# pkuyzy/TLC-GNN

Measured on NVIDIA B200. Metric: vicinity_pd_pi_per_sec, higher is better.
Workload: dtype f64

## Files before the change

### tlc-gnn_b200/csrc/k1t_sssp_table.cu

```cuda
#include <cstdlib>

#include <cstdio>
#include <cstring>

#include "tlc_common.cuh"

namespace tlc {
namespace {

__global__ void sssp_mark_kernel(const int32_t* __restrict__ targets, int64_t E, int node_mode, GraphView g, SsspTables tb) {
  const int64_t total = 2 * E;
  for (int64_t i = blockIdx.x * (int64_t)blockDim.x + threadIdx.x; i < total; i += (int64_t)gridDim.x * blockDim.x) {
    if (node_mode && (i & 1)) continue;
    const int32_t x = targets[i];
    if (x < 0 || x >= g.N || g.rowptr[x + 1] == g.rowptr[x]) continue;
    if (tb.state[x] == 0 && atomicCAS(&tb.state[x], 0, 1) == 0) tb.list[atomicAdd(tb.count, 1)] = x;
  }
}

__global__ void sssp_mark_all_kernel(GraphView g, SsspTables tb) {
  for (int x = blockIdx.x * blockDim.x + threadIdx.x; x < g.N; x += gridDim.x * blockDim.x) {
    if (g.rowptr[x + 1] == g.rowptr[x]) continue;
    if (tb.state[x] == 0 && atomicCAS(&tb.state[x], 0, 1) == 0) tb.list[atomicAdd(tb.count, 1)] = x;
  }
}

constexpr int BQ = 2048;
struct BuildShared {
  int32_t q[BQ];
  int32_t qn, qhead;
  unsigned long long dmin;
  int32_t any;
};

__global__ void __launch_bounds__(1024) sssp_build_kernel(GraphView g, SsspTables tb, const uint32_t* __restrict__ ball_cache,
                                                          const float* __restrict__ gminw, double* __restrict__ pw_scratch,
                                                          int plain) {
  extern __shared__ __align__(16) unsigned long long bsm[];
  __shared__ BuildShared sh;
  const int N = g.N, W = (N + 31) / 32;
  const int tid = threadIdx.x, nt = blockDim.x, lane = tid & 31, wid = tid >> 5, nw = nt >> 5;
  unsigned long long* dist = bsm;
  int32_t* par = reinterpret_cast<int32_t*>(bsm + N);
  uint32_t* ball = reinterpret_cast<uint32_t*>(par + N);
  uint8_t* state = reinterpret_cast<uint8_t*>(ball + W);
  double* pw = pw_scratch + (size_t)blockIdx.x * N;
  const int cnt = *tb.count;
  for (int idx = blockIdx.x; idx < cnt; idx += gridDim.x) {
    const int32_t root = tb.list[idx];
    __syncthreads();
    for (int x = tid; x < N; x += nt) { dist[x] = INF_BITS; state[x] = 0; par[x] = -1; }
    for (int w = tid; w < W; w += nt) ball[w] = ball_cache[(size_t)root * W + w];
    __syncthreads();
    if (tid == 0) { dist[root] = 0ull; state[root] = 1; }
    __syncthreads();
    for (int phase = 0; phase < 2 * N + 2; phase++) {
      if (tid == 0) { sh.dmin = INF_BITS; sh.qn = 0; sh.qhead = 0; }
      __syncthreads();
      unsigned long long lm = INF_BITS;
      for (int x = tid; x < N; x += nt) if (state[x] == 1) { const unsigned long long d = dist[x]; lm = d < lm ? d : lm; }
      lm = warp_min_u64(lm);
      if (lane == 0 && lm != INF_BITS) atomicMin(&sh.dmin, lm);
      __syncthreads();
      const unsigned long long dminb = sh.dmin;
      if (dminb == INF_BITS) break;
      const double dmin = __longlong_as_double((long long)dminb);
      for (int x = tid; x < N; x += nt) {
        if (state[x] != 1) continue;
        if (__longlong_as_double((long long)dist[x]) <= __dadd_rn(dmin, (double)gminw[x])) {
          const int pos = atomicAdd(&sh.qn, 1);
          if (pos < BQ) { state[x] = 2; sh.q[pos] = x; }
        }
      }
      __syncthreads();
      const int qn = min(sh.qn, BQ);
      for (;;) {
        int i = 0;
        if (lane == 0) i = atomicAdd(&sh.qhead, 1);
        i = __shfl_sync(0xffffffffu, i, 0);
        if (i >= qn) break;
        const int x = sh.q[i];
        const double dx = __longlong_as_double((long long)dist[x]);
        const int a = g.rowptr[x], b = g.rowptr[x + 1];
        for (int e = a + lane; e < b; e += 32) {
          const int y = g.col[e];
          if (!test_bit(ball, y)) continue;
          const unsigned long long tbv = (unsigned long long)__double_as_longlong(__dadd_rn(dx, __dadd_rn(g.kappa[e], 1.0)));
          if (tbv < dist[y]) { atomicMin(&dist[y], tbv); if (state[y] == 0) state[y] = 1; }
        }
      }
      __syncthreads();
    }
    __syncthreads();
    for (int x = wid; x < N; x += nw) {
      const unsigned long long dxb = dist[x];
      if (x == root || dxb == INF_BITS) continue;
      const int a = g.rowptr[x], b = g.rowptr[x + 1];
      for (int e0 = a; e0 < b; e0 += 32) {
        const int e = e0 + lane;
        bool hit = false;
        double w = 0.0;
        int y = 0;
        if (e < b) {
          y = g.col[e];
          w = __dadd_rn(g.kappa[e], 1.0);
          const unsigned long long dyb = dist[y];
          hit = dyb != INF_BITS && (unsigned long long)__double_as_longlong(__dadd_rn(__longlong_as_double((long long)dyb), w)) == dxb;
        }
        const unsigned bal = __ballot_sync(0xffffffffu, hit);
        if (bal) {
          if (lane == __ffs(bal) - 1) { par[x] = y; pw[x] = w; }
          break;
        }
      }
    }
    __threadfence_block();
    __syncthreads();
    double* Drow = tb.D + (size_t)root * N;
    double* Qrow = tb.Q + (size_t)root * N;
    int32_t* Prow = tb.P + (size_t)root * N;
    double* Wrow = tb.PW + (size_t)root * N;
    for (int x = tid; x < N; x += nt) {
      const unsigned long long dxb = dist[x];
      Drow[x] = __longlong_as_double((long long)dxb);
      Prow[x] = par[x];
      Wrow[x] = par[x] >= 0 ? pw[x] : 0.0;
      double res;
      if (x == root) res = 0.0;
      else if (dxb == INF_BITS || par[x] < 0) res = NO_PATH_DIST;
      else {
        PySum ps{0.0, 0.0, 0};
        int y = x, guard = 0;
        while (y != root && guard++ <= N) { pysum_add(ps, pw[y], plain != 0); y = par[y]; }
        res = pysum_get(ps, plain != 0);
      }
      Qrow[x] = res;
    }
    __syncthreads();
    if (tid == 0) { __threadfence(); tb.state[root] = 2; }
  }
}

struct TableShared {
  double redd[32];
  int32_t wsum[33];
  int32_t ninv;
  int32_t nextra;
  int32_t dinv;
  int32_t nia;
  int32_t any;
};
#ifdef T1_PROFILE
__device__ unsigned long long g_t1prof[24];
#define TPROF(i) do { if (tid == 0) { const long long tnow_ = clock64(); atomicAdd(&g_t1prof[i], (unsigned long long)(tnow_ - tprev_)); tprev_ = tnow_; } } while (0)
#else
#define TPROF(i) do { } while (0)
#endif


__global__ void __launch_bounds__(1024) filtration_table_kernel(Params p, ChunkView c, int t0, int cap, GraphView g,
                                                                const uint32_t* __restrict__ ball_cache, SsspTables tb, int W) {
  extern __shared__ __align__(16) unsigned long long dynt[];
  __shared__ TableShared sh;
  const int t = t0 + blockIdx.x;
  const int tid = threadIdx.x, nt = blockDim.x, lane = tid & 31, wid = tid >> 5, nw = nt >> 5;
  const bool node_mode = p.mode == TLC_MODE_NODE;
  const int64_t vo = c.voff[t];
  const int N = g.N;
  unsigned long long* dist = dynt;
  uint16_t* parl = reinterpret_cast<uint16_t*>(dynt + cap);
  uint8_t* cls = reinterpret_cast<uint8_t*>(parl + cap);
  uint32_t* bm = reinterpret_cast<uint32_t*>(reinterpret_cast<unsigned char*>(dynt) + (size_t)cap * 11);
  uint16_t* lid = reinterpret_cast<uint16_t*>(bm + 2 * W);

#ifdef T1_PROFILE
  long long tprev_ = clock64();
#endif
  const int64_t ti = c.tidx[t];
  const int32_t u = c.tgt[2 * ti], v = c.tgt[2 * ti + 1];
  if (unknown_target(g, u, v, node_mode)) {
    if (tid == 0) { c.tn[t] = 0; c.tnp[t] = 0; c.tnpos[t] = 0; c.tnneg[t] = 0; c.tlu[t] = -1; c.tlv[t] = -1;
                    c.tstatus[t] = TLC_ST_UNKNOWN_NODE; }
    return;
  }
  const int n = graph_row_bitmap(c, t, ball_cache, W, u, v, node_mode, bm, sh.wsum);
  {
    uint32_t* l32 = reinterpret_cast<uint32_t*>(lid);
    for (int i = tid; i < (N + 1) / 2; i += nt) l32[i] = 0xffffffffu;
  }
  __syncthreads();
  for (int w = wid; w < W; w += nw) {
    const uint32_t bits = bm[w];
    if (!((bits >> lane) & 1u)) continue;
    const int lx = (int)bm[W + w] + __popc(bits & lanemask_lt());
    const int32_t x = w * 32 + lane;
    const int32_t ra = g.rowptr[x];
    c.vert[vo + lx] = x;
    c.astart[vo + lx] = ra;
    c.adeg[vo + lx] = g.rowptr[x + 1] - ra;
    lid[x] = (uint16_t)lx;
  }
  const int lu = bitmap_rank(bm, W, u);
  const int lv = node_mode ? lu : bitmap_rank(bm, W, v);
  uint8_t st0 = (lu >= 0 && lv >= 0) ? TLC_ST_OK : TLC_ST_TRIVIAL;
  if (n == 0 || (node_mode && n == 1)) st0 = TLC_ST_EMPTY;
  if (tid == 0) {
    c.tn[t] = n; c.tlu[t] = lu; c.tlv[t] = lv; c.tstatus[t] = st0;
    if (c.count_m) c.tm[t] = 0;
    c.tnp[t] = 0; c.tnpos[t] = 0; c.tnneg[t] = 0; c.tncls[t] = 0;
  }
  __syncthreads();
      TPROF(0);
  if (n == 0 || st0 > TLC_ST_TRIVIAL) return;

  const int32_t* __restrict__ vert = c.vert + vo;
  double* d1 = c.d1 + vo;
  double* d2 = c.d2 + vo;
  double* fval = c.fval + vo;
  int32_t* hint = c.neg + vo;
  int32_t* hint0 = c.vcls + vo;
  int32_t* inv = c.vs0 + vo;
  int32_t* extra = c.vs1 + vo;
  int32_t* bpos = c.vs2 + vo;
  uint32_t* iap = reinterpret_cast<uint32_t*>(c.vord + vo);
  int32_t* iaq = c.vrank + vo;
  uint2* ia2 = reinterpret_cast<uint2*>(c.v64a + vo);
  uint2* ia3 = reinterpret_cast<uint2*>(c.v64c + vo);
  uint2* ia4 = reinterpret_cast<uint2*>(c.fval + vo);
  const bool roots_in = lu >= 0 && lv >= 0;
  const bool plain = (p.flags & TLC_F_SUM_PLAIN) != 0;
  const bool two = roots_in && !node_mode && lu != lv;
  constexpr uint8_t UNKNOWN = 0, VALID = 1, INVALID = 2, UNREACH = 3;

  if (!roots_in) {
    for (int x = tid; x < n; x += nt) { d1[x] = NO_PATH_DIST; d2[x] = NO_PATH_DIST; hint[x] = -1; hint0[x] = -1; }
  } else {
    for (int r = 0; r < (two ? 2 : 1); r++) {
      const int root = r == 0 ? lu : lv;
      const int32_t groot = r == 0 ? u : v;
      const double* __restrict__ Drow = tb.D + (size_t)groot * N;
      const double* __restrict__ Qrow = tb.Q + (size_t)groot * N;
      const double* __restrict__ Wrow = tb.PW + (size_t)groot * N;
      const int32_t* __restrict__ Prow = tb.P + (size_t)groot * N;
      double* out = r == 0 ? d1 : d2;
      int32_t* hnt = r == 0 ? hint0 : hint;
      if (tid == 0) { sh.ninv = 0; sh.nextra = 0; sh.dinv = 0; sh.nia = 0; }
      for (int x = tid; x < n; x += nt) {
        const int32_t gx = vert[x];
        uint8_t cl;
        uint16_t pl = 0xffff;
        if (x == root) cl = VALID;
        else {
          const int32_t gp = Prow[gx];
          pl = gp >= 0 ? lid[gp] : (uint16_t)0xffff;
          cl = pl == 0xffff ? INVALID : UNKNOWN;
        }
        cls[x] = cl; parl[x] = pl;
        dist[x] = (unsigned long long)__double_as_longlong(Drow[gx]);
        if (r == 0) { hint[x] = -1; hint0[x] = -1; }
      }
      __syncthreads();
      TPROF(1);
      for (int round = 0; round <= n; round++) {
        int ch = 0;
        for (int x = tid; x < n; x += nt) {
          if (cls[x] != UNKNOWN) continue;
          const uint8_t pc = cls[parl[x]];
          if (pc != UNKNOWN) { cls[x] = pc; ch = 1; }
          else ch = 1;
        }
        if (!__syncthreads_or(ch)) break;
      }
      TPROF(2);
      for (int x0 = 0; x0 < n; x0 += nt) {
        const int x = x0 + tid;
        const bool iv = x < n && cls[x] == INVALID;
        const unsigned bal = __ballot_sync(0xffffffffu, iv);
        int base = 0;
        if (bal && lane == 0) base = atomicAdd(&sh.ninv, __popc(bal));
        base = __shfl_sync(0xffffffffu, base, 0);
        if (iv) {
          const int32_t gx = vert[x];
          inv[base + __popc(bal & lanemask_lt())] = x;
          dist[x] = INF_BITS; bpos[x] = 0x7fffffff;
          atomicAdd(&sh.dinv, g.rowptr[gx + 1] - g.rowptr[gx]);
        }
      }
      __syncthreads();
      TPROF(3);
      const int ninv = sh.ninv;
      int chunk = min(512, max(32, ((sh.dinv / (nt / 2) + 31) / 32) * 32));
      while (sh.dinv / chunk > n / 2) chunk *= 2;
      for (int i = tid; i < ninv; i += nt) {
        const int32_t gx = vert[inv[i]];
        const int cnt = (g.rowptr[gx + 1] - g.rowptr[gx] + chunk - 1) / chunk;
        if (cnt > 1) {
          const int at = atomicAdd(&sh.nextra, cnt - 1);
          for (int j = 1; j < cnt; j++) extra[at + j - 1] = (inv[i] << 12) | j;
        }
      }
      __syncthreads();
      TPROF(4);
      const int nextra = sh.nextra, nitems = ninv + nextra;
      const int l8 = lane & 7, grp = tid >> 3, ngrp = nt >> 3;
      const unsigned gm = 0xffu << (lane & 24);
      constexpr int ITEM_RESCAN = 1 << 30;
      auto item_bounds = [&](int i, int& x, int& a, int& b, bool flagged_only) {
        const int raw = i < ninv ? inv[i] : extra[i - ninv];
        const int pk = i < ninv ? ((raw & 0xffff) << 12) : (raw & (ITEM_RESCAN - 1));
        x = pk >> 12;
        const int ra = c.astart[vo + x];
        a = ra + (pk & 4095) * chunk;
        b = min(ra + c.adeg[vo + x], a + chunk);
        if (flagged_only && !(raw & ITEM_RESCAN)) b = a;
      };
      auto ia_put = [&](int k, uint32_t pr, int pos) {
        if (k < n) { iap[k] = pr; iaq[k] = pos; }
        else if (k < 2 * n) ia2[k - n] = make_uint2(pr, (uint32_t)pos);
        else if (k < 3 * n) ia3[k - 2 * n] = make_uint2(pr, (uint32_t)pos);
        else if (k < 4 * n) ia4[k - 3 * n] = make_uint2(pr, (uint32_t)pos);
      };
      auto ia_get = [&](int k, uint32_t& pr, int& pos) {
        if (k < n) { pr = iap[k]; pos = iaq[k]; return; }
        const uint2 v2 = k < 2 * n ? ia2[k - n] : k < 3 * n ? ia3[k - 2 * n] : ia4[k - 3 * n];
        pr = v2.x; pos = (int)v2.y;
      };
      const int capw = (4 * n) / nw;
      int cntw = 0;
      auto relax_rows = [&](bool first) -> int {
        int ch = 0;
        for (int kb = 0; kb * ngrp < nitems; kb += 8) {
          int mx = 0, ma = 0, mb = 0;
          { const int itl = (kb + l8) * ngrp + grp; if (itl < nitems) item_bounds(itl, mx, ma, mb, !first); }
          for (int j = 0; j < 8; j++) {
            const int x = __shfl_sync(gm, mx, j, 8), a = __shfl_sync(gm, ma, j, 8), b = __shfl_sync(gm, mb, j, 8);
            int trips = (b - a + 31) >> 5;
            trips = max(trips, __shfl_xor_sync(0xffffffffu, trips, 8));
            trips = max(trips, __shfl_xor_sync(0xffffffffu, trips, 16));
            unsigned long long best = INF_BITS;
            for (int t5 = 0; t5 < trips; t5++) {
              const int e0 = a + l8 + 32 * t5;
              uint4 rc[4];
// ... 55 lines not shown
          ewt[i] = __hiloint2double((int)rc.w, (int)rc.z);
        }
      }
#ifdef T1_PROFILE
      long long tlr0_ = clock64();
      int nrounds_ = 0;
#endif
      for (int round = 1; round <= ninv + 1; round++) {
        int ch = 0;
#ifdef T1_PROFILE
        nrounds_++;
#endif
#pragma unroll
        for (int i = 0; i < 4; i++) {
          if (epr[i] == 0xffffffffu) continue;
          const int x = (int)(epr[i] >> 16), ly = (int)(epr[i] & 0xffffu);
          const unsigned long long dyb = dist[ly], dxb = dist[x];
          if (dyb != INF_BITS) {
            const unsigned long long cand = (unsigned long long)__double_as_longlong(__dadd_rn(__longlong_as_double((long long)dyb), ewt[i]));
            if (cand < dxb && cand < atomicMin(&dist[x], cand)) ch = 1;
          }
          if (dxb != INF_BITS) {
            const unsigned long long c2 = (unsigned long long)__double_as_longlong(__dadd_rn(__longlong_as_double((long long)dxb), ewt[i]));
            if (c2 < dyb && c2 < atomicMin(&dist[ly], c2)) ch = 1;
          }
        }
        for (int k = lane + 128; k < nlist; k += 32) {
          uint32_t pr; int pos;
          ia_get(wid * capw + k, pr, pos);
          const int x = (int)(pr >> 16), ly = (int)(pr & 0xffffu);
          const unsigned long long dyb = dist[ly], dxb = dist[x];
          if (dyb == INF_BITS && dxb == INF_BITS) continue;
          const uint4 rc = __ldg(g.rec + pos);
          const double w = __hiloint2double((int)rc.w, (int)rc.z);
          if (dyb != INF_BITS) {
            const unsigned long long cand = (unsigned long long)__double_as_longlong(__dadd_rn(__longlong_as_double((long long)dyb), w));
            if (cand < dxb && cand < atomicMin(&dist[x], cand)) ch = 1;
          }
          if (dxb != INF_BITS) {
            const unsigned long long c2 = (unsigned long long)__double_as_longlong(__dadd_rn(__longlong_as_double((long long)dxb), w));
            if (c2 < dyb && c2 < atomicMin(&dist[ly], c2)) ch = 1;
          }
        }
        if (full) ch |= relax_rows(false);
        if (!__syncthreads_or(ch)) break;
      }
      TPROF(6);
#ifdef T1_PROFILE
      if (lane == 0) atomicAdd(&g_t1prof[15], (unsigned long long)cntw);
      if (tid == 0) { atomicAdd(&g_t1prof[17], (unsigned long long)nrounds_); if (full) atomicAdd(&g_t1prof[16], (unsigned long long)(clock64() - tlr0_)); }
      if (tid == 0) { atomicAdd(&g_t1prof[11], (unsigned long long)(full ? 1 : 0)); atomicAdd(&g_t1prof[12], 1ull); atomicAdd(&g_t1prof[13], (unsigned long long)nitems); atomicAdd(&g_t1prof[14], (unsigned long long)sh.dinv); }
#endif
      for (int kb = 0; kb * ngrp < nitems; kb += 8) {
        int mx = 0, ma = 0, mb = 0;
        { const int itl = (kb + l8) * ngrp + grp; if (itl < nitems) item_bounds(itl, mx, ma, mb, false); }
        for (int j = 0; j < 8; j++) {
        const int x = __shfl_sync(gm, mx, j, 8), a = __shfl_sync(gm, ma, j, 8);
        int b = __shfl_sync(gm, mb, j, 8);
        const unsigned long long dxb = b > a ? dist[x] : INF_BITS;
        if (dxb == INF_BITS) b = a;
        int hit = 0x7fffffff;
        for (int e0 = a; e0 < b; e0 += 32) {
          uint4 rc[4];
#pragma unroll
          for (int q = 0; q < 4; q++) rc[q] = e0 + l8 + 8 * q < b ? __ldg(g.rec + e0 + l8 + 8 * q) : make_uint4(0xffffffffu, 0u, 0u, 0u);
#pragma unroll
          for (int q = 3; q >= 0; q--) {
            if (rc[q].x == 0xffffffffu) continue;
            const uint16_t ly = lid[rc[q].x];
            if (ly == 0xffff) continue;
            const unsigned long long dyb = dist[ly];
            if (dyb != INF_BITS && (unsigned long long)__double_as_longlong(__dadd_rn(__longlong_as_double((long long)dyb), __hiloint2double((int)rc[q].w, (int)rc[q].z))) == dxb)
              hit = e0 + l8 + 8 * q;
          }
          if (__ballot_sync(gm, hit != 0x7fffffff)) break;
        }
#pragma unroll
        for (int o = 4; o; o >>= 1) hit = min(hit, __shfl_xor_sync(gm, hit, o));
        if (l8 == 0 && hit != 0x7fffffff) atomicMin(&bpos[x], hit);
        }
      }
      __syncthreads();
      TPROF(7);
      for (int x = tid; x < n; x += nt) {
        unsigned long long wb = 0;
        if (x != root) {
          if (cls[x] == VALID) wb = (unsigned long long)__double_as_longlong(Wrow[vert[x]]);
          else {
            const int pos = bpos[x];
            if (dist[x] != INF_BITS && pos != 0x7fffffff) {
              const uint4 rc = __ldg(g.rec + pos);
              parl[x] = lid[rc.x];
              wb = ((unsigned long long)rc.w << 32) | rc.z;
            } else cls[x] = UNREACH;
          }
        }
        dist[x] = wb;
      }
      __syncthreads();
      TPROF(8);
      for (int x = tid; x < n; x += nt) {
        double res;
        const uint8_t cl = cls[x];
        if (x == root) res = 0.0;
        else if (cl == VALID) { res = Qrow[vert[x]]; hnt[x] = (int32_t)parl[x]; }
        else if (cl == UNREACH) res = NO_PATH_DIST;
        else {
          hnt[x] = (int32_t)parl[x];
          PySum ps{0.0, 0.0, 0};
          int y = x, guard = 0;
          while (y != root && guard++ <= n) {
            const int py = (int)parl[y];
            pysum_add(ps, __longlong_as_double((long long)dist[y]), plain);
            y = py;
          }
          res = pysum_get(ps, plain);
        }
        out[x] = res;
      }
      __syncthreads();
      TPROF(9);
    }
    if (!two) for (int x = tid; x < n; x += nt) d2[x] = d1[x];
    __syncthreads();
    if (tid == 0) zero_roots(d1, d2, lu, lv);
  }
  __syncthreads();

  double mx = -1.0, sm = -1.0;
  for (int x = tid; x < n; x += nt) {
    const double a = d1[x], b = d2[x];
    mx = fmax(mx, fv_descriptor(TLC_DESC_MAX, node_mode, a, b));
    sm = fmax(sm, fv_descriptor(TLC_DESC_SUM, node_mode, a, b));
  }
  double smax = block_reduce_max(mx, sh.redd);
  double ssum = block_reduce_max(sm, sh.redd);
  const bool norm = (p.flags & TLC_F_NORM) != 0;
  if (norm && !fv_normalisers(p.flags, smax, ssum)) {
    if (tid == 0) c.tstatus[t] = TLC_ST_DEGENERATE;
    return;
  }
  for (int x = tid; x < n; x += nt) fval[x] = fv_value(p.descriptor, node_mode, norm, smax, ssum, d1[x], d2[x]);
  TPROF(10);
}

}

void launch_sssp_build(const GraphView& g, const Params& p, const int32_t* targets, int64_t E, const SsspTables& tb,
                       const uint32_t* ball_cache, const float* gminw, double* pw_scratch, int grid, cudaStream_t st) {
  if (!tb.D) return;
  cudaMemsetAsync(tb.count, 0, sizeof(int), st);
  if (targets) {
    if (E <= 0) return;
    const int mgrid = (int)std::min<int64_t>((2 * E + 255) / 256, 4096);
    sssp_mark_kernel<<<mgrid, 256, 0, st>>>(targets, E, p.mode == TLC_MODE_NODE ? 1 : 0, g, tb);
  } else {
    sssp_mark_all_kernel<<<(g.N + 255) / 256, 256, 0, st>>>(g, tb);
  }
  count_launch();
  const size_t bytes = sssp_build_smem(g.N);
  cudaFuncSetAttribute((const void*)sssp_build_kernel, cudaFuncAttributeMaxDynamicSharedMemorySize, (int)bytes);
  cudaFuncSetAttribute((const void*)sssp_build_kernel, cudaFuncAttributePreferredSharedMemoryCarveout, cudaSharedmemCarveoutMaxShared);
  sssp_build_kernel<<<grid, 1024, bytes, st>>>(g, tb, ball_cache, gminw, pw_scratch, (p.flags & TLC_F_SUM_PLAIN) ? 1 : 0);
  count_launch();
}

size_t sssp_build_smem(int N) { return (size_t)N * (8 + 4 + 1) + (size_t)(N + 31) / 32 * 4 + 16; }

void launch_filtration_table(const GraphView& g, const Params& p, const ChunkView& c, const VicinityScratch& vs,
                             const SsspTables& tb, int t0, int cnt, int block, int64_t n_max, cudaStream_t st) {
  const int W = (g.N + 31) / 32;
  const int cap = (int)((n_max + 7) / 8 * 8);
  const size_t bytes = (size_t)cap * 11 + (size_t)2 * W * 4 + ((size_t)g.N + 1) / 2 * 4 + 16;
  if (block < 128) block = 128;
  if (bytes + sizeof(TableShared) > 110 * 1024 && block >= 512) block = 1024;
  if (const char* env = getenv("TLC_TABLE_BLOCK")) block = atoi(env);
  cudaFuncSetAttribute((const void*)filtration_table_kernel, cudaFuncAttributeMaxDynamicSharedMemorySize, (int)bytes);
  cudaFuncSetAttribute((const void*)filtration_table_kernel, cudaFuncAttributePreferredSharedMemoryCarveout, cudaSharedmemCarveoutMaxShared);
#ifdef T1_PROFILE
  if (getenv("T1_PROFILE_DUMP")) {
    unsigned long long h[24];
    cudaMemcpyFromSymbol(h, g_t1prof, sizeof h);
    static const char* nm[11] = {"prologue", "class_init", "class_rounds", "compaction", "chunks", "first_round", "later_rounds",
                                 "tree_rule", "parents", "path_sums", "descriptors"};
    unsigned long long tot = 0;
    for (int i = 0; i < 11; i++) tot += h[i];
    if (tot) {
      fprintf(stderr, "[1t profile]");
      for (int i = 0; i < 11; i++) fprintf(stderr, " %s %.1f%%", nm[i], 100.0 * (double)h[i] / (double)tot);
      fprintf(stderr, " | total %.1f Mticks | roots %llu, with flagged chunks %llu, items/root %.0f, records/root %.0f, list entries/root %.0f\n", (double)tot / 1e6,
              h[12], h[11], (double)h[13] / (double)(h[12] ? h[12] : 1), (double)h[14] / (double)(h[12] ? h[12] : 1), (double)h[15] / (double)(h[12] ? h[12] : 1));
      fprintf(stderr, "[1t profile] later rounds per root %.2f; ticks of the later rounds spent in roots with flagged chunks: %.1f Mticks\n", (double)h[17] / (double)(h[12] ? h[12] : 1), (double)h[16] / 1e6);
    }
    memset(h, 0, sizeof h);
    cudaMemcpyToSymbol(g_t1prof, h, sizeof h);
  }
#endif
  filtration_table_kernel<<<cnt, block, bytes, st>>>(p, c, t0, cap, g, vs.ball_cache, tb, W);
  count_launch();
}

// ... 8 lines not shown
```

### tlc-gnn_b200/csrc/tlc_api.cu

```cuda
#include <algorithm>
#include <atomic>
#include <cstdio>
#include <cstdlib>
#include <cmath>
#include <cstring>
#include <numeric>
#include <string>
#include <vector>

#include "tlc_common.cuh"

namespace tlc {
static std::atomic_llong g_launches{0};
int64_t launch_count() { return g_launches.load(); }
void count_launch() { g_launches.fetch_add(1); }
}

using namespace tlc;

static thread_local std::string g_err;
static int fail(int rc, const std::string& msg) {
  g_err = msg;
  return rc;
}
// ... 53 lines not shown
    for (int i = 0; i < 4; i++) small_rows[i] += o.small_rows[i];
    chunks += o.chunks; live += o.live; sum_n += o.sum_n; sum_m += o.sum_m; handed_back += o.handed_back;
    general += o.general; rowcheck += o.rowcheck; blocks += o.blocks; direct += o.direct; table += o.table;
    bytes += o.bytes;
    return *this;
  }
};

static cudaError_t grow_keep(DevBuf& b, size_t used, size_t need, cudaStream_t st) {
  if (b.p && need <= b.bytes) return cudaSuccess;
  DevBuf nb;
  cudaError_t e = nb.reserve(need);
  if (e == cudaSuccess && used) e = cudaMemcpyAsync(nb.p, b.p, used, cudaMemcpyDeviceToDevice, st);
  if (e == cudaSuccess) e = cudaStreamSynchronize(st);
  if (e == cudaSuccess) b = std::move(nb);
  return e;
}

struct PairBufs {
  DevBuf kind, bv, dv, birth, death;
  int64_t cap = 0;
  DiagArea view() const {
    return DiagArea{kind.as<uint8_t>(), bv.as<int32_t>(), dv.as<int32_t>(), birth.as<double>(), death.as<double>()};
  }
  cudaError_t grow(int64_t used, int64_t need, cudaStream_t st) {
    if (need <= cap && kind.p) return cudaSuccess;
    const int64_t n = std::max<int64_t>(need, cap + cap / 2);
    cudaError_t e = cudaSuccess;
    DevBuf* bufs[5] = {&kind, &bv, &dv, &birth, &death};
    const size_t sz[5] = {1, 4, 4, 8, 8};
    for (int i = 0; i < 5 && e == cudaSuccess; i++) e = grow_keep(*bufs[i], (size_t)used * sz[i], (size_t)n * sz[i] + 16, st);
    if (e == cudaSuccess) cap = n;
    return e;
  }
};

struct DiagCollect {
  bool on = false;
  DevBuf np, soff, poff;
  PairBufs small, staged, out;
  int64_t small_total = 0, staged_used = 0;
  DevBuf chunk;
};

struct tlc_graph {
  int device = 0;
  GraphView gv{};
  DevBuf rowptr, col, kappa, rec;
  cudaStream_t stream = nullptr, own_stream = nullptr;
  cudaStream_t side[3] = {nullptr, nullptr, nullptr};
  cudaEvent_t ev_fork = nullptr, ev_join[3] = {nullptr, nullptr, nullptr};
  DevBuf arena;
  size_t arena_req = 0;
  DevBuf bitmaps, queue;
  DevBuf ball_cache, ball_acc, ball_state, ball_list;
  int vic_grid = 0, vic_hop = -1;
  DevBuf work_counter;
  ChunkView detail_chunk{};
  DevBuf gminw;
  int probe_hop = -1, probe_mode = -1, probe_age = 0;
  bool probe_direct = false;
  DevBuf d_n, d_m, d_ds, d_st, d_bytes;
  int64_t call_cap = 0;
  DevBuf io_t, io_pi, io_st;
  int64_t io_cap_t = 0, io_cap_pi = 0;
  PinBuf h_pin;
  CallStats last;
  DevBuf sm_list_b, sm_list_c, sm_list_big, sm_list_b2;
  cudaStream_t small_stream2 = nullptr;
  cudaEvent_t ev_small_c = nullptr;
  cudaStream_t small_stream = nullptr;
  cudaEvent_t ev_small_a = nullptr, ev_small_bc = nullptr;
  DevBuf sm_sub;
  DevBuf sm_idx;
  DevBuf sm_pi;
  DevBuf sm_pi32, sm_st;
  int64_t sm_cap = 0, sm_sub_cap = 0;
  DevBuf sm_dev;
  PinBuf sm_host;
  int small_skip = 0;
  int small_hop = -1, small_mode = -1;
  double hks_time = 0.1;
  SsspTables sssp{};
  DevBuf sssp_D, sssp_Q, sssp_P, sssp_PW, sssp_state, sssp_list, sssp_count, sssp_pw;
  int sssp_plain = -1, sssp_hop = -1;
  bool sssp_tried = false, sssp_all = false;
  double sssp_build_ms = 0;
  DevBuf peer_own;
  int64_t peer_rows = 0;
  int peer_r2 = 0;
  PeerTables peers{};
  std::vector<void*> peer_opened;
  unsigned int peer_epoch = 0;
  DevBuf peer_ticket;
  DevBuf px_pi32, px_pi, px_st;
  int64_t px_cap = 0;
  std::vector<cudaEvent_t> ev_pool;
  int sm_count = 0;
  DiagCollect dg;

  ~tlc_graph() {
    for (void* q : peer_opened) cudaIpcCloseMemHandle(q);
    for (cudaStream_t s : {own_stream, side[0], side[1], side[2], small_stream, small_stream2})
      if (s) cudaStreamDestroy(s);
    for (cudaEvent_t e : {ev_fork, ev_join[0], ev_join[1], ev_join[2], ev_small_a, ev_small_bc, ev_small_c})
      if (e) cudaEventDestroy(e);
    for (cudaEvent_t e : ev_pool) cudaEventDestroy(e);
  }
};

static int ensure_call_buffers(tlc_graph* g, int64_t E) {
  if (E <= g->call_cap) return TLC_OK;
  const size_t cap = (size_t)(E + E / 8 + 1024);
  CK(g->d_n.reserve(cap * 4));
  CK(g->d_m.reserve(cap * 4));
  CK(g->d_ds.reserve(cap * 4));
  CK(g->d_st.reserve(cap));
  CK(g->d_bytes.reserve(cap * 8));
  g->call_cap = (int64_t)cap;
  return TLC_OK;
}

static int ensure_io_buffers(tlc_graph* g, int64_t E, int r2) {
  const int64_t cap = E + E / 8 + 1024;
  if (E > g->io_cap_t) {
    CK(g->io_t.reserve((size_t)cap * 8));
    CK(g->io_st.reserve((size_t)cap));
    g->io_cap_t = cap;
  }
  if (E * r2 > g->io_cap_pi) {
    CK(g->io_pi.reserve((size_t)cap * r2 * 8));
    g->io_cap_pi = cap * r2;
  }
  return TLC_OK;
}

static size_t arena_limit(const tlc_graph* g) {
  if (g->arena_req) return g->arena_req;
  const char* env = getenv("TLC_ARENA_GB");
  return (size_t)((env ? atof(env) : 24.0) * (double)(1ull << 30));
}

static int ensure_arena(tlc_graph* g, size_t need_min, size_t need_all) {
  const size_t limit = arena_limit(g);
  if (g->arena.p && g->arena.bytes >= need_min && g->arena.bytes >= std::min(need_all, limit)) return TLC_OK;
  size_t free_b = 0, total_b = 0;
  CK(cudaMemGetInfo(&free_b, &total_b));
  const size_t had = g->arena.bytes;
  free_b += had;
  g->arena.release();
  size_t want = std::max(std::min(limit, need_all + need_all / 2), need_min);
  want = std::max(want, std::min(limit, std::max<size_t>(2 * had, (size_t)256 << 20)));
  const size_t cap = (size_t)((double)free_b * 0.85);
  if (want > cap) want = cap;
  if (want < need_min)
    return fail(TLC_E_NOMEM, "one vicinity needs " + std::to_string(need_min) + " arena bytes, only " +
                                 std::to_string(cap) + " available");
  CK(g->arena.reserve(want));
  return TLC_OK;
}

static VicinityScratch make_vs(const tlc_graph* g) {
  return VicinityScratch{g->bitmaps.as<uint32_t>(), g->queue.as<int32_t>(), g->vic_grid, g->ball_cache.as<uint32_t>(),
                         g->ball_acc.as<unsigned long long>(), g->ball_state.as<int32_t>(), g->ball_list.as<int32_t>(),
                         g->work_counter.as<int>() + 2};
}

static int ensure_vicinity_scratch(tlc_graph* g, const Params& p) {
  if (g->vic_hop == p.hop && g->vic_grid > 0) return TLC_OK;
  for (DevBuf* b : {&g->bitmaps, &g->queue, &g->ball_cache, &g->ball_acc, &g->ball_state, &g->ball_list}) b->release();
  {
    const char* env = getenv("TLC_BALL_CACHE_GB");
    const double gb = env ? atof(env) : 16.0;
    const size_t Wc = ((size_t)g->gv.N + 31) / 32;
    const size_t need = (size_t)g->gv.N * Wc * sizeof(uint32_t);
    size_t free_b = 0, total_b = 0;
    cudaMemGetInfo(&free_b, &total_b);
    if (gb > 0 && (double)need <= gb * (double)(1ull << 30) && need <= free_b / 4) {
      CK(g->ball_cache.reserve(std::max<size_t>(need, 16)));
      CK(g->ball_acc.reserve((size_t)g->gv.N * 2 * sizeof(unsigned long long)));
      CK(g->ball_state.reserve((size_t)g->gv.N * sizeof(int32_t)));
      CK(g->ball_list.reserve((size_t)g->gv.N * sizeof(int32_t)));
      CK(cudaMemset(g->ball_state.p, 0, (size_t)g->gv.N * sizeof(int32_t)));
    }
  }
  size_t W = 0;
  bool smem = false;
  g->vic_grid = vicinity_grid(g->device, g->gv, p, &W, &smem);
  if (!smem) CK(g->bitmaps.reserve((size_t)g->vic_grid * 2 * W * sizeof(uint32_t)));
  if (p.hop > 2) CK(g->queue.reserve((size_t)g->vic_grid * 2 * (size_t)g->gv.N * sizeof(int32_t)));
  g->vic_hop = p.hop;
  return TLC_OK;
}

static int prepare_call(tlc_graph* g, const Params& p, int64_t E) {
  int rc = ensure_call_buffers(g, E);
  return rc ? rc : ensure_vicinity_scratch(g, p);
}

static int ensure_sssp_tables(tlc_graph* g, const Params& p) {
  const int plain = (p.flags & TLC_F_SUM_PLAIN) ? 1 : 0;
  if (!g->sssp_tried) {
    g->sssp_tried = true;
    const char* env = getenv("TLC_SSSP_CACHE_GB");
    const double gb = env ? atof(env) : 8.0;
    const size_t N = (size_t)g->gv.N;
    const size_t need = N * N * 28;
    size_t free_b = 0, total_b = 0;
    cudaMemGetInfo(&free_b, &total_b);
    if (gb > 0 && N <= 16384 && (double)need <= gb * (double)(1ull << 30) && need <= free_b / 3 &&
        sssp_build_smem((int)N) <= 227 * 1024) {
      CK(g->sssp_D.reserve(N * N * 8));
      CK(g->sssp_Q.reserve(N * N * 8));
      CK(g->sssp_P.reserve(N * N * 4));
      CK(g->sssp_PW.reserve(N * N * 8));
      CK(g->sssp_state.reserve(N * 4));
      CK(g->sssp_list.reserve(N * 4));
      CK(g->sssp_count.reserve(64));
      CK(g->sssp_pw.reserve((size_t)g->sm_count * N * 8));
      CK(cudaMemset(g->sssp_state.p, 0, N * 4));
      g->sssp = SsspTables{g->sssp_D.as<double>(), g->sssp_Q.as<double>(), g->sssp_P.as<int32_t>(), g->sssp_PW.as<double>(),
                           g->sssp_state.as<int32_t>(), g->sssp_list.as<int32_t>(), g->sssp_count.as<int>()};
      g->sssp_plain = plain;
      g->sssp_hop = p.hop;
    }
  }
  if (g->sssp.D && (g->sssp_plain != plain || g->sssp_hop != p.hop)) {
    CK(cudaMemsetAsync(g->sssp.state, 0, (size_t)g->gv.N * 4, g->stream));
    g->sssp_plain = plain;
    g->sssp_hop = p.hop;
    g->sssp_all = false;
  }
  return TLC_OK;
}

static size_t chunk_bytes(int64_t T, int64_t Nv, int64_t Ne, int64_t Na, int64_t Wd = 0) {
  const int64_t Np = Nv + Ne + T;
  return (size_t)(Nv * BV + Ne * BE + Na * BA + Np * BP + (T + 1) * BT + T * Wd * 8) + ALIGN * 60;
}

template <typename T_>
static T_* take(char*& cur, int64_t count) {
  T_* p = reinterpret_cast<T_*>(cur);
  cur += align_up((size_t)count * sizeof(T_));
  return p;
}

static ChunkView carve(char* arena, int64_t T, int64_t Nv, int64_t Ne, int64_t Na, const int32_t* d_targets,
                       int64_t Wd = 0) {
  ChunkView c{};
  char* cur = arena;
  const int64_t Np = Nv + Ne + T;
  c.T = (int32_t)T;
  c.tgt = d_targets;
  c.tidx = take<int64_t>(cur, T);
  c.voff = take<int64_t>(cur, T + 1);
  c.eoff = take<int64_t>(cur, T + 1);
  c.aoff = take<int64_t>(cur, T + 1);
  c.tn = take<int32_t>(cur, T); c.tm = take<int32_t>(cur, T); c.tlu = take<int32_t>(cur, T); c.tlv = take<int32_t>(cur, T);
  c.tnp = take<int32_t>(cur, T); c.tnpos = take<int32_t>(cur, T); c.tnneg = take<int32_t>(cur, T); c.tncls = take<int32_t>(cur, T);
  c.tnb = take<int32_t>(cur, T); c.tminv = take<int32_t>(cur, T); c.tmaxv = take<int32_t>(cur, T);
  c.tstatus = take<uint8_t>(cur, T);
  c.tfb = take<uint8_t>(cur, T);
  c.vord = take<int32_t>(cur, Nv); c.vrank = take<int32_t>(cur, Nv);
  c.bfirst = take<int32_t>(cur, Nv + T);
  c.astart = take<int32_t>(cur, Nv); c.adeg = take<int32_t>(cur, Nv); c.aminw = take<float>(cur, Nv);
  c.anb = take<uint32_t>(cur, Na); c.aw = take<double>(cur, Na);
  c.vert = take<int32_t>(cur, Nv); c.vcls = take<int32_t>(cur, Nv); c.vs0 = take<int32_t>(cur, Nv);
  c.vs1 = take<int32_t>(cur, Nv); c.vs2 = take<int32_t>(cur, Nv); c.neg = take<int32_t>(cur, Nv);
  c.fval = take<double>(cur, Nv); c.d1 = take<double>(cur, Nv); c.d2 = take<double>(cur, Nv);
  c.v64a = take<unsigned long long>(cur, Nv); c.v64b = take<unsigned long long>(cur, Nv);
  c.v64c = take<unsigned long long>(cur, Nv);
  c.elo = take<int32_t>(cur, Ne); c.ehi = take<int32_t>(cur, Ne); c.pos = take<int32_t>(cur, Ne);
  c.arank = take<int32_t>(cur, Ne);
  c.ew = take<double>(cur, Ne);
  c.ord_asc = take<uint32_t>(cur, Ne); c.ord_desc = take<uint32_t>(cur, Ne);
  c.sp0 = take<uint32_t>(cur, Ne); c.sp1 = take<uint32_t>(cur, Ne);
  c.sk0 = take<unsigned long long>(cur, Ne); c.sk1 = take<unsigned long long>(cur, Ne);
  c.isneg = take<uint8_t>(cur, Ne);
  c.pkind = take<uint8_t>(cur, Np);
  c.pbv = take<int32_t>(cur, Np); c.pdv = take<int32_t>(cur, Np);
  c.pbirth = take<double>(cur, Np); c.pdeath = take<double>(cur, Np);
  c.dbm = Wd > 0 ? take<uint32_t>(cur, T * 2 * Wd) : nullptr;
  c.W = (int32_t)Wd;
  return c;
}

static int block_for(int64_t m_max) {
  if (m_max >= 32768) return 512;
  if (m_max >= 4096) return 256;
  if (m_max >= 512) return 128;
  if (m_max >= 96) return 64;
  return 32;
}
static int size_class(int64_t m) { return block_for(m); }
static int smem_class(int64_t n) { return n > 22000 ? 0 : (n > 16000 ? 1 : 2); }

struct StageTimer {
  bool on;
  cudaStream_t st;
  std::vector<cudaEvent_t>* pool;
  size_t used, first;
  std::vector<int> stage;
  StageTimer(cudaStream_t s, std::vector<cudaEvent_t>* pool_, size_t start) : st(s), pool(pool_), used(start), first(start) {
// ... 1446 lines not shown
```

### tlc-gnn_b200/csrc/tlc_common.cuh

```cuda
#pragma once
#include <cuda_runtime.h>
#include <stdint.h>

#include "../../include/tlc_b200.h"

namespace tlc {

struct GraphView {
  int32_t N;
  int64_t nnz;
  const int32_t* rowptr;
  const int32_t* col;
  const double* kappa;
  const uint4* rec;
};

struct ChunkView {
  int32_t T;
  const int32_t* tgt;
  const int64_t* tidx;
  const int64_t* voff;
  const int64_t* eoff;
  const int64_t* aoff;
  int32_t *tn, *tm, *tlu, *tlv, *tnp, *tnpos, *tnneg, *tncls;
// ... 207 lines not shown
}
__device__ __forceinline__ bool fv_normalisers(uint32_t flags, double& smax, double& ssum) {
  if (flags & TLC_F_NORM_EPS) { smax = __dadd_rn(smax, 1e-10); ssum = __dadd_rn(ssum, 1e-10); return true; }
  return !(smax == 0.0 || ssum == 0.0);
}
__device__ __forceinline__ double fv_value(int descriptor, bool node_mode, bool norm, double smax, double ssum, double a,
                                           double b) {
  double f = fv_descriptor(descriptor, node_mode, a, b);
  if (norm) f = __ddiv_rn(f, descriptor == TLC_DESC_SUM ? ssum : smax);
  return f;
}

template <typename PT>
__device__ __forceinline__ int uf_find(PT* p, int x) {
  for (;;) {
    const int px = (int)p[x];
    if (px == x) return x;
    const int gp = (int)p[px];
    p[x] = (PT)gp;
    x = gp;
  }
}

__device__ __forceinline__ double norm_cdf(double x) {
  return erfc(-x / 1.4142135623730951) * 0.5;
}
__device__ __forceinline__ double ramp_weight(double pers) {
  return pers < 0.0 ? 0.0 : (pers > 1.0 ? 1.0 : pers);
}
__device__ __forceinline__ void cdf_diffs(int res, double step, double birth, double pers, double* gb, double* gp) {
  double pb = norm_cdf(0.0 - birth), pp = norm_cdf(0.0 - pers);
#pragma unroll
  for (int i = 1; i <= res; i++) {
    const double pt = i * step;
    const double cb = norm_cdf(pt - birth), cp = norm_cdf(pt - pers);
    gb[i - 1] = cb - pb; gp[i - 1] = cp - pp;
    pb = cb; pp = cp;
  }
}

struct VicinityScratch {
  uint32_t* bitmaps;
  int32_t* queue;
  int grid;
  uint32_t* ball_cache;
  unsigned long long* ball_acc;
  int32_t* ball_state;
  int32_t* ball_list;
  int* ball_count;
};

void launch_vicinity_sizes(const GraphView& g, const Params& p, const int32_t* targets, int64_t E, int32_t* out_n,
                           int32_t* out_m, int32_t* out_ds, uint8_t* out_status, double* out_bytes,
                           const VicinityScratch& vs, int* work_counter, cudaStream_t st);
void launch_vicinity_light(const GraphView& g, const Params& p, const int32_t* targets, int64_t E, int32_t* out_n,
                           int32_t* out_m, int32_t* out_ds, uint8_t* out_status, double* out_bytes,
                           const VicinityScratch& vs, int sm_count, cudaStream_t st);
void launch_vicinity_fill(const GraphView& g, const Params& p, const ChunkView& c, const VicinityScratch& vs,
                          int* work_counter, cudaStream_t st);
void launch_filtration(const Params& p, const ChunkView& c, int t0, int cnt, int block, int64_t n_max, cudaStream_t st);
void launch_degree_filtration(const Params& p, const ChunkView& c, cudaStream_t st);
void launch_hks_filtration(const Params& p, const ChunkView& c, double t, int64_t n_max, cudaStream_t st);
void launch_filtration_direct(const GraphView& g, const Params& p, const ChunkView& c, const VicinityScratch& vs,
                              const float* gminw, int t0, int cnt, int block, int64_t n_max, cudaStream_t st);
void launch_edgelist(const Params& p, const ChunkView& c, int block, int fb_only, cudaStream_t st);
void launch_sort(const Params& p, const ChunkView& c, int block, int sweep_mask, int fb_only, cudaStream_t st);
void launch_union_find(const Params& p, const ChunkView& c, int block, int smem_ints, int build_lists, int sweep_mask,
                       int fb_only, cudaStream_t st);
void launch_vorder(const Params& p, const ChunkView& c, int t0, int cnt, int block, int64_t n_max, cudaStream_t st);
void launch_sweep(const Params& p, const ChunkView& c, int t0, int cnt, int64_t n_max, cudaStream_t st);
void launch_loops(const Params& p, const ChunkView& c, int block, int smem_ints, int64_t n_max, cudaStream_t st);
void launch_pimg(const Params& p, const ChunkView& c, double* out_pi, float* out_pi_f32, uint8_t* out_status,
                 int block, cudaStream_t st);
void launch_pimg_single(const double* dgm, int64_t K, int res, double* out, cudaStream_t st);

void launch_gather_rows(const double* table, int64_t rows, int r2, const int64_t* index, int64_t start, int64_t n,
                        float* out, int* bad, int sm_count, cudaStream_t st);

void launch_scatter_rows(const double* src_pi, const float* src_pi32, const uint8_t* src_st, const int64_t* idx, int64_t k,
                         int r2, double* dst_pi, float* dst_pi32, uint8_t* dst_st, int sm_count, cudaStream_t st);

struct SsspTables {
  double* D;
  double* Q;
  int32_t* P;
  double* PW;
  int32_t* state;
  int32_t* list;
  int* count;
};
void launch_sssp_build(const GraphView& g, const Params& p, const int32_t* targets, int64_t E, const SsspTables& tb,
                       const uint32_t* ball_cache, const float* gminw, double* pw_scratch, int grid, cudaStream_t st);
size_t sssp_build_smem(int N);
void launch_filtration_table(const GraphView& g, const Params& p, const ChunkView& c, const VicinityScratch& vs,
                             const SsspTables& tb, int t0, int cnt, int block, int64_t n_max, cudaStream_t st);
size_t filtration_table_smem(int N, int64_t n_max);

void launch_ricci(const int32_t* rowptr, const int32_t* col, const uint32_t* ball1, const uint32_t* ball2, int W,
                  const int64_t* epos, const int64_t* emir, const int32_t* esrc, int64_t E, double alpha, const double* kval4,
                  const double* wsum, double wnb, int topk, int max_iter, double stop_thr, int cap, bool codes_smem,
                  uint8_t* slab, size_t slab_stride, int grid, double* out, int32_t* iters, cudaStream_t st);
size_t ricci_smem_bytes(int cap, bool codes_smem);

struct SmallDiag {
  const int64_t* poff;
  int32_t* np;
  uint8_t* kind;
  int32_t *bv, *dv;
  double *birth, *death;
  int graph_ids = 0;
  int want_desc = 1;
};
struct SmallStats {
  unsigned long long handled[3];
  unsigned long long live, sum_n, sum_m;
  double bytes;
};
void launch_small(const GraphView& g, const Params& p, const int32_t* targets, int64_t E, const VicinityScratch& vs,
                  double* out_pi, float* out_pi32, uint8_t* out_status, int32_t* list_b, int32_t* list_c, int32_t* list_big,
                  int* counters, int32_t* out_n, int32_t* out_m, const SmallDiag* diag, SmallStats* stats, int sm_count,
                  int phases, cudaStream_t st, int32_t* list_b2 = nullptr);
void launch_gather_targets(const int32_t* targets, const int32_t* list, int64_t k, int32_t* sub, int64_t* idx, cudaStream_t st);

struct DiagArea {
  uint8_t* kind;
  int32_t *bv, *dv;
  double *birth, *death;
};
__host__ __device__ inline int diag_pairs(uint8_t status, int32_t np) {
  return (status <= TLC_ST_TRIVIAL || status == TLC_ST_NO_TREE_EDGES) && np > 0 ? np : 0;
}
void launch_export_pairs(const ChunkView& c, const int64_t* dst, const int64_t* rows, const DiagArea& area,
                         int64_t area_base, int32_t* np_out, int64_t* soff_out, int sm_count, cudaStream_t st);
void launch_scan_counts(const int32_t* np, int64_t E, int64_t* poff, cudaStream_t st);
void launch_gather_pairs(const int32_t* np, const int64_t* soff, const int64_t* poff, int64_t E, const DiagArea& a,
                         const DiagArea& b, int64_t split_at, const DiagArea& out, int sm_count, cudaStream_t st);

constexpr int PEER_MAX = 16;
constexpr size_t PEER_HEADER_BYTES = 256;
struct PeerTables {
  int n;
  void* table[PEER_MAX];
};
void launch_peer_scatter(const float* src_pi32, const uint8_t* src_st, const int64_t* row_index, int64_t k, int r2,
                         const PeerTables& pt, unsigned int* ticket, int sm_count, cudaStream_t st);
void launch_peer_wait(const unsigned int* flag, unsigned int target, cudaStream_t st);

int64_t launch_count();
void count_launch();
int vicinity_grid(int device, const GraphView& g, const Params& p, size_t* bitmap_words, bool* use_smem);
void launch_ball_cache(const GraphView& g, const Params& p, const int32_t* targets, int64_t E, const VicinityScratch& vs,
                       cudaStream_t st);

}
```

Measured before the change: 749,200.

## Interleave SSSP Q and PW tables into double2 and restrict path sums to invalid vertices

Merges the separate per-root Q and PW tables into one interleaved double2 array, so the filtration kernel fetches both values with a single 16-byte gather. The table-setup and fixup loops are unrolled by four to batch the independent global gathers. The final path-sum pass now walks only the invalid-vertex list instead of every vertex, with valid results written in the earlier pass. It also adds a minBlocks=1 launch bound to the build kernel, and the interleaved layout keeps total memory the same.

After: 807,800, median of 6. +7.8%, better.

```diff
diff --git a/tlc-gnn_b200/csrc/k1t_sssp_table.cu b/tlc-gnn_b200/csrc/k1t_sssp_table.cu
--- a/tlc-gnn_b200/csrc/k1t_sssp_table.cu
+++ b/tlc-gnn_b200/csrc/k1t_sssp_table.cu
@@ -33,7 +33,7 @@
   int32_t any;
 };
 
-__global__ void __launch_bounds__(1024) sssp_build_kernel(GraphView g, SsspTables tb, const uint32_t* __restrict__ ball_cache,
+__global__ void __launch_bounds__(1024, 1) sssp_build_kernel(GraphView g, SsspTables tb, const uint32_t* __restrict__ ball_cache,
                                                           const float* __restrict__ gminw, double* __restrict__ pw_scratch,
                                                           int plain) {
   extern __shared__ __align__(16) unsigned long long bsm[];
@@ -117,24 +117,23 @@
     __threadfence_block();
     __syncthreads();
     double* Drow = tb.D + (size_t)root * N;
-    double* Qrow = tb.Q + (size_t)root * N;
     int32_t* Prow = tb.P + (size_t)root * N;
-    double* Wrow = tb.PW + (size_t)root * N;
+    double2* QWrow = tb.QW + (size_t)root * N;
     for (int x = tid; x < N; x += nt) {
       const unsigned long long dxb = dist[x];
-      Drow[x] = __longlong_as_double((long long)dxb);
-      Prow[x] = par[x];
-      Wrow[x] = par[x] >= 0 ? pw[x] : 0.0;
+      const int32_t px = par[x];
       double res;
       if (x == root) res = 0.0;
-      else if (dxb == INF_BITS || par[x] < 0) res = NO_PATH_DIST;
+      else if (dxb == INF_BITS || px < 0) res = NO_PATH_DIST;
       else {
         PySum ps{0.0, 0.0, 0};
         int y = x, guard = 0;
         while (y != root && guard++ <= N) { pysum_add(ps, pw[y], plain != 0); y = par[y]; }
         res = pysum_get(ps, plain != 0);
       }
-      Qrow[x] = res;
+      Drow[x] = __longlong_as_double((long long)dxb);
+      Prow[x] = px;
+      QWrow[x] = make_double2(res, px >= 0 ? pw[x] : 0.0);
     }
     __syncthreads();
     if (tid == 0) { __threadfence(); tb.state[root] = 2; }
@@ -239,25 +238,35 @@
       const int root = r == 0 ? lu : lv;
       const int32_t groot = r == 0 ? u : v;
       const double* __restrict__ Drow = tb.D + (size_t)groot * N;
-      const double* __restrict__ Qrow = tb.Q + (size_t)groot * N;
-      const double* __restrict__ Wrow = tb.PW + (size_t)groot * N;
       const int32_t* __restrict__ Prow = tb.P + (size_t)groot * N;
+      const double2* __restrict__ QWrow = tb.QW + (size_t)groot * N;
       double* out = r == 0 ? d1 : d2;
       int32_t* hnt = r == 0 ? hint0 : hint;
       if (tid == 0) { sh.ninv = 0; sh.nextra = 0; sh.dinv = 0; sh.nia = 0; }
-      for (int x = tid; x < n; x += nt) {
-        const int32_t gx = vert[x];
-        uint8_t cl;
-        uint16_t pl = 0xffff;
-        if (x == root) cl = VALID;
-        else {
-          const int32_t gp = Prow[gx];
-          pl = gp >= 0 ? lid[gp] : (uint16_t)0xffff;
-          cl = pl == 0xffff ? INVALID : UNKNOWN;
-        }
-        cls[x] = cl; parl[x] = pl;
-        dist[x] = (unsigned long long)__double_as_longlong(Drow[gx]);
-        if (r == 0) { hint[x] = -1; hint0[x] = -1; }
+      for (int x0 = tid; x0 < n; x0 += 4 * nt) {
+        int32_t gx4[4];
+#pragma unroll
+        for (int k = 0; k < 4; k++) { const int x = x0 + k * nt; gx4[k] = x < n ? vert[x] : -1; }
+        double d4[4];
+        int32_t p4[4];
+#pragma unroll
+        for (int k = 0; k < 4; k++) { d4[k] = gx4[k] >= 0 ? Drow[gx4[k]] : 0.0; p4[k] = gx4[k] >= 0 ? Prow[gx4[k]] : -1; }
+#pragma unroll
+        for (int k = 0; k < 4; k++) {
+          const int x = x0 + k * nt;
+          if (x >= n) continue;
+          uint8_t cl;
+          uint16_t pl = 0xffff;
+          if (x == root) cl = VALID;
+          else {
+            const int32_t gp = p4[k];
+            pl = gp >= 0 ? lid[gp] : (uint16_t)0xffff;
+            cl = pl == 0xffff ? INVALID : UNKNOWN;
+          }
+          cls[x] = cl; parl[x] = pl;
+          dist[x] = (unsigned long long)__double_as_longlong(d4[k]);
+          if (r == 0) { hint[x] = -1; hint0[x] = -1; }
+        }
       }
       __syncthreads();
       TPROF(1);
@@ -479,41 +488,52 @@
       }
       __syncthreads();
       TPROF(7);
-      for (int x = tid; x < n; x += nt) {
-        unsigned long long wb = 0;
-        if (x != root) {
-          if (cls[x] == VALID) wb = (unsigned long long)__double_as_longlong(Wrow[vert[x]]);
-          else {
+      for (int x0 = tid; x0 < n; x0 += 4 * nt) {
+        int32_t gx4[4];
+#pragma unroll
+        for (int k = 0; k < 4; k++) {
+          const int x = x0 + k * nt;
+          gx4[k] = x < n && x != root && cls[x] == VALID ? vert[x] : -1;
+        }
+        double2 e4[4];
+#pragma unroll
+        for (int k = 0; k < 4; k++) e4[k] = gx4[k] >= 0 ? QWrow[gx4[k]] : make_double2(0.0, 0.0);
+#pragma unroll
+        for (int k = 0; k < 4; k++) {
+          const int x = x0 + k * nt;
+          if (x >= n) continue;
+          unsigned long long wb = 0;
+          if (x == root) out[x] = 0.0;
+          else if (gx4[k] >= 0) {
+            wb = (unsigned long long)__double_as_longlong(e4[k].y);
+            out[x] = e4[k].x;
+            hnt[x] = (int32_t)parl[x];
+          } else {
             const int pos = bpos[x];
             if (dist[x] != INF_BITS && pos != 0x7fffffff) {
               const uint4 rc = __ldg(g.rec + pos);
-              parl[x] = lid[rc.x];
+              const uint16_t pl = lid[rc.x];
+              parl[x] = pl;
+              hnt[x] = (int32_t)pl;
               wb = ((unsigned long long)rc.w << 32) | rc.z;
-            } else cls[x] = UNREACH;
-          }
-        }
-        dist[x] = wb;
+            } else { cls[x] = UNREACH; out[x] = NO_PATH_DIST; }
+          }
+          dist[x] = wb;
+        }
       }
       __syncthreads();
       TPROF(8);
-      for (int x = tid; x < n; x += nt) {
-        double res;
-        const uint8_t cl = cls[x];
-        if (x == root) res = 0.0;
-        else if (cl == VALID) { res = Qrow[vert[x]]; hnt[x] = (int32_t)parl[x]; }
-        else if (cl == UNREACH) res = NO_PATH_DIST;
-        else {
-          hnt[x] = (int32_t)parl[x];
-          PySum ps{0.0, 0.0, 0};
-          int y = x, guard = 0;
-          while (y != root && guard++ <= n) {
-            const int py = (int)parl[y];
-            pysum_add(ps, __longlong_as_double((long long)dist[y]), plain);
-            y = py;
-          }
-          res = pysum_get(ps, plain);
-        }
-        out[x] = res;
+      for (int i = tid; i < ninv; i += nt) {
+        const int x = inv[i] & 0xffff;
+        if (cls[x] == UNREACH) continue;
+        PySum ps{0.0, 0.0, 0};
+        int y = x, guard = 0;
+        while (y != root && guard++ <= n) {
+          const int py = (int)parl[y];
+          pysum_add(ps, __longlong_as_double((long long)dist[y]), plain);
+          y = py;
+        }
+        out[x] = pysum_get(ps, plain);
       }
       __syncthreads();
       TPROF(9);
diff --git a/tlc-gnn_b200/csrc/tlc_api.cu b/tlc-gnn_b200/csrc/tlc_api.cu
--- a/tlc-gnn_b200/csrc/tlc_api.cu
+++ b/tlc-gnn_b200/csrc/tlc_api.cu
@@ -159,7 +159,7 @@
   int small_hop = -1, small_mode = -1;
   double hks_time = 0.1;
   SsspTables sssp{};
-  DevBuf sssp_D, sssp_Q, sssp_P, sssp_PW, sssp_state, sssp_list, sssp_count, sssp_pw;
+  DevBuf sssp_D, sssp_P, sssp_QW, sssp_state, sssp_list, sssp_count, sssp_pw;
   int sssp_plain = -1, sssp_hop = -1;
   bool sssp_tried = false, sssp_all = false;
   double sssp_build_ms = 0;
@@ -282,21 +282,20 @@
     const char* env = getenv("TLC_SSSP_CACHE_GB");
     const double gb = env ? atof(env) : 8.0;
     const size_t N = (size_t)g->gv.N;
-    const size_t need = N * N * 28;
+    const size_t need = N * N * (8 + 4 + 16);
     size_t free_b = 0, total_b = 0;
     cudaMemGetInfo(&free_b, &total_b);
     if (gb > 0 && N <= 16384 && (double)need <= gb * (double)(1ull << 30) && need <= free_b / 3 &&
         sssp_build_smem((int)N) <= 227 * 1024) {
       CK(g->sssp_D.reserve(N * N * 8));
-      CK(g->sssp_Q.reserve(N * N * 8));
       CK(g->sssp_P.reserve(N * N * 4));
-      CK(g->sssp_PW.reserve(N * N * 8));
+      CK(g->sssp_QW.reserve(N * N * 16));
       CK(g->sssp_state.reserve(N * 4));
       CK(g->sssp_list.reserve(N * 4));
       CK(g->sssp_count.reserve(64));
       CK(g->sssp_pw.reserve((size_t)g->sm_count * N * 8));
       CK(cudaMemset(g->sssp_state.p, 0, N * 4));
-      g->sssp = SsspTables{g->sssp_D.as<double>(), g->sssp_Q.as<double>(), g->sssp_P.as<int32_t>(), g->sssp_PW.as<double>(),
+      g->sssp = SsspTables{g->sssp_D.as<double>(), g->sssp_P.as<int32_t>(), g->sssp_QW.as<double2>(),
                            g->sssp_state.as<int32_t>(), g->sssp_list.as<int32_t>(), g->sssp_count.as<int>()};
       g->sssp_plain = plain;
       g->sssp_hop = p.hop;
diff --git a/tlc-gnn_b200/csrc/tlc_common.cuh b/tlc-gnn_b200/csrc/tlc_common.cuh
--- a/tlc-gnn_b200/csrc/tlc_common.cuh
+++ b/tlc-gnn_b200/csrc/tlc_common.cuh
@@ -313,9 +313,8 @@
 
 struct SsspTables {
   double* D;
-  double* Q;
   int32_t* P;
-  double* PW;
+  double2* QW;
   int32_t* state;
   int32_t* list;
   int* count;
```
